# kekeliu-whu/MSF_LOAM

Measured on AMD Instinct MI355X. Metric: scan-to-map registrations/s, higher is better.
Workload: dtype f64 (f32 kNN distances)

## Files before the change

msf_loam_amd/csrc/msfl_api.hip:

```cpp
#include <hip/hip_runtime.h>
#include <rocprim/device/device_radix_sort.hpp>
#include <rocprim/device/device_scan.hpp>
#include <rocprim/device/device_select.hpp>

#include <algorithm>
#include <cmath>
#include <cstdio>
#include <cstdlib>
#include <cstring>
#include <functional>
#include <utility>
#include <chrono>
#include <string>
#include <vector>

#include <condition_variable>
#include <mutex>
#include <thread>

#include "../../include/msfl_c_api.h"
#include "msfl_kernels.cuh"
#include "msfl_extract.cuh"
#include "msfl_odom.cuh"
#include "msfl_grid.cuh"
// ... 163 lines not shown
  DevBuf rec;
  DevBuf d2, nn;
  DevBuf scan;
};

enum TimerClass { T_ASSOC = 0, T_SOLVE, T_INDEX, T_EXTRACT, T_ODOM, T_FIT, T_ASSOC_SEEDED , T_COUNT };

struct TimedSpan { hipEvent_t a, b; int cls; };

struct RejectOptions {
  int mode = MSFL_REJECT_OFF;
  double thr2 = 0.0, fraction = 0.0;
  int which = MSFL_REJECT_LAST_OUTER;
};
struct RegOptions {
  double unc_min_eig = 0.0;
  int degen_on = 0;
  double degen_min_eig = 0.0;
  RejectOptions rej;
};
struct RecordSink {
  void* out = nullptr;
  int capacity = 0;
  msfl_mem mem = MSFL_MEM_HOST;
  DevBuf dev;
  void set(const void* p, int n, msfl_mem m) { out = const_cast<void*>(p); capacity = p ? n : 0; mem = m; }
  bool host() const { return out && mem == MSFL_MEM_HOST; }
};

}

struct msfl_handle_s {
  int device = 0;
  hipStream_t own_stream = nullptr;
  hipStream_t stream = nullptr;
  msfl_params prm{};
  std::string last_error;

  bool have_map = false;
  MapIndex map_c, map_s;
  int grid_cap_cells = 64 * 1024 * 1024;
  int h2d_chunk_scans = 512;
  int h2d_sub_chunks = 2;
  int solve_records_block = 0;
  int vox_nonfinite_cloud = -1;
  const float4* vox_staged_pts = nullptr;
  bool voxel_no_big = false;
  int odom_bin_split = -1;
  int prep_split = -1;
  bool voxel_force_global = false;
  long long odom_wave_max_targets = -1;
  bool odom_force_brute = false;
  int knn_form = 0;

  DevBuf in_corner, in_surf, in_off, poses, status, info, records, pprime, nn;
  std::vector<int> in_off_host; const void* in_off_host_ptr = nullptr;
  DevBuf idx_cell_of, idx_count, idx_scanned, idx_bbox, idx_cub, idx_stage;
  bool index_single = false;
  DevBuf knn_count;
  size_t idx_count_zero = 0;
  DeskewScratch dk;
  ExtractScratch ex;
  OdomScratch od;
  VoxelScratch vox;
  PointPassScratch pp;
  PairScratch pr;
  ScoreScratch sc;

  RegOptions opt;
  RecordSink unc, degen, rej, prior;
  DevBuf rej_keys;

  PinRing pin;
  PinBuf readback;
  hipStream_t copy_stream = nullptr;
  hipEvent_t copy_ev[9] = {};

  int timing = 0;
  std::vector<TimedSpan> spans;
  std::vector<hipEvent_t> free_events;
  double t_ms[T_COUNT] = {0};
  int t_n[T_COUNT] = {0};
};

namespace {

msfl_status fail(msfl_handle* h, msfl_status s, const std::string& msg) {
  if (h) h->last_error = msg;
  return s;
}

#define HIPCHK(h, expr)                                                                            \
  do {                                                                                             \
    hipError_t e__ = (expr);                                                                       \
    if (e__ != hipSuccess)                                                                         \
      return fail(h, MSFL_HIP_ERROR, std::string(#expr) + ": " + hipGetErrorString(e__));          \
  } while (0)

msfl_status fail(msfl_places* p, msfl_status s, const std::string& msg);

template <class H, class T>
msfl_status stage_in(H* h, DevBuf& buf, const void* src, size_t n, msfl_mem mem, hipStream_t st, T** d) {
  if (mem != MSFL_MEM_HOST) { *d = static_cast<T*>(const_cast<void*>(src)); return MSFL_OK; }
  HIPCHK(h, buf.reserve(std::max<size_t>(1, n) * sizeof(T)));
  if (n > 0) HIPCHK(h, hipMemcpyAsync(buf.p, src, n * sizeof(T), hipMemcpyHostToDevice, st));
  *d = buf.as<T>();
// ... 302 lines not shown
  }
  const size_t span = (size_t)j.cap[0] + 1 + (size_t)j.cap[1] + 1;
  HIPCHK(h, h->idx_cell_of.reserve(((size_t)n_c + (size_t)n_s) * sizeof(int)));
  const void* count_before = h->idx_count.p;
  HIPCHK(h, h->idx_count.reserve(span * sizeof(int)));
  if (h->idx_count.p != count_before) h->idx_count_zero = 0;
  HIPCHK(h, h->idx_scanned.reserve(span * sizeof(int)));
  j.cell_of = h->idx_cell_of.as<int>(); j.count = h->idx_count.as<int>(); j.scanned = h->idx_scanned.as<int>();
  j.blocks0 = div_up(n_c, 256); j.bbox_blocks0 = std::min(div_up(n_c, 1024), 256);
  j.radius = std::sqrt((double)h->prm.map_knn_max_sq_dist);
  const int bbox_blocks1 = std::min(div_up(n_s, 1024), 256), blocks1 = div_up(n_s, 256);
  hipLaunchKernelGGL(grid_bbox_pair_kernel, dim3(j.bbox_blocks0 + bbox_blocks1), dim3(256), 0, st, j);
  const size_t zeroed = h->idx_count_zero;
  h->idx_count_zero = 0;
  if (span > zeroed) HIPCHK(h, hipMemsetAsync(h->idx_count.p, 0, span * sizeof(int), st));
  hipLaunchKernelGGL(grid_count_pair_kernel, dim3(j.blocks0 + blocks1), dim3(256), 0, st, j);
  size_t tmp_bytes = 0;
  HIPCHK(h, rocprim::exclusive_scan(nullptr, tmp_bytes, j.count, j.scanned, 0, span, rocprim::plus<int>(), st));
  HIPCHK(h, h->idx_cub.reserve(tmp_bytes));
  HIPCHK(h, rocprim::exclusive_scan(h->idx_cub.p, tmp_bytes, j.count, j.scanned, 0, span, rocprim::plus<int>(), st));
  hipLaunchKernelGGL(grid_scatter_pair_kernel, dim3(j.blocks0 + blocks1), dim3(256), 0, st, j);
  HIPCHK(h, hipGetLastError());
  h->idx_count_zero = std::max(zeroed, span);
  return MSFL_OK;
}

template <class Kernel, class... Tail>
void launch_knn5(msfl_handle* h, Kernel kernel, dim3 grid, dim3 block, const BatchView& bv, const double* d_poses, const int* d_status,
                 Tail... tail) {
  hipLaunchKernelGGL(kernel, grid, block, 0, h->stream, bv, d_poses, d_status,
                     (const GridDesc*)h->map_c.gdesc.as<GridDesc>(), h->map_c.sorted.as<float4>(), h->map_c.cell_start.as<int>(),
                     (const GridDesc*)h->map_s.gdesc.as<GridDesc>(), h->map_s.sorted.as<float4>(), h->map_s.cell_start.as<int>(),
                     (const int*)h->map_c.pos_of.as<int>(), (const int*)h->map_s.pos_of.as<int>(), h->prm.map_knn_max_sq_dist, tail...);
}

bool assoc_whole_batch(const msfl_handle* h, const BatchView& bv, bool deskew, int n_rec, const double* full) {
  return !deskew && !bv.dyn && n_rec >= 65536 && !full && h->timing != 3;
}

void s_launch_assoc(msfl_handle* h, const BatchView& bv_all, const double* d_poses, const int* d_status, bool deskew,
                    const DeskewView& dv, int n_rec, double* full = nullptr, int rec_begin = 0, int rec_end = -1, bool second_pass = false) {
  const bool whole_batch = rec_end < 0 && assoc_whole_batch(h, bv_all, deskew, n_rec, full);
  hipStream_t st = h->stream;
  int* nn = h->nn.as<int>();
  BatchView bv = bv_all;
  if (rec_end >= 0) { bv.rec_begin = rec_begin; bv.n_records = rec_end; n_rec = rec_end - rec_begin; }
  if (n_rec <= 0) return;
  const dim3 grid(div_up(n_rec, kAssocBlock)), block(kAssocBlock);
  {
    ScopedTimer timer(h, second_pass ? T_ASSOC_SEEDED : T_ASSOC);
    if (h->timing == 3) {
      unsigned long long* cnt = h->knn_count.as<unsigned long long>();
      if (deskew) launch_knn5(h, knn5_scan2map_kernel<true, true>, grid, block, bv, d_poses, d_status, dv, nn, cnt, nullptr, nullptr);
      else launch_knn5(h, knn5_scan2map_kernel<false, true>, grid, block, bv, d_poses, d_status, dv, nn, cnt + (second_pass ? 1 : 0), nullptr, nullptr);
    } else if (whole_batch) {
      const int n_s = bv.n_surf_total, n_c = n_rec - n_s;
      const int edge_blocks = div_up(n_c, kAssocBlock), plane_blocks = div_up(n_s, kAssocBlock);
      launch_knn5(h, knn5_scan2map_split_kernel, dim3(edge_blocks + plane_blocks), block, bv, d_poses, d_status, nn, h->records.as<double>(), edge_blocks);
    } else if (!deskew && (h->knn_form == 2 || (h->knn_form == 0 && (n_rec <= kKnnRowsMaxRecords ||
                                                                       (bv.dyn && n_rec <= 8 * kKnnRowsMaxRecords)))))
      launch_knn5(h, knn5_scan2map_rows_kernel, dim3(div_up(n_rec, kKnnRowsBlock / kKnnRowLanes)), dim3(kKnnRowsBlock), bv, d_poses, d_status, nn);
    else if (deskew)
      launch_knn5(h, knn5_scan2map_kernel<true>, grid, block, bv, d_poses, d_status, dv, nn, nullptr, nullptr, nullptr);
    else
      launch_knn5(h, knn5_scan2map_kernel<false>, grid, block, bv, d_poses, d_status, dv, nn, nullptr, nullptr, nullptr);
  }
  {
    ScopedTimer timer(h, T_FIT);
    if (deskew)
      hipLaunchKernelGGL(fit_scan2map_kernel<true>, grid, block, 0, st, bv, h->map_c.sorted.as<float4>(),
                         h->map_s.sorted.as<float4>(), (const int*)nn, h->prm.line_eigen_ratio, h->prm.plane_tolerance, dv,
                         h->records.as<double>(), full);
    else
      if (whole_batch) {
        const int n_c = n_rec - bv.n_surf_total, n_s = bv.n_surf_total;
        const int edge_blocks = div_up(n_c, kAssocBlock), plane_blocks = div_up(n_s, kAssocBlock);
        hipLaunchKernelGGL(fit_scan2map_split_kernel, dim3(edge_blocks + plane_blocks), block, 0, st, bv, h->map_c.sorted.as<float4>(),
                           h->map_s.sorted.as<float4>(), (const int*)nn, h->prm.line_eigen_ratio, h->prm.plane_tolerance, dv,
                           h->records.as<double>(), full, edge_blocks);
      } else
      hipLaunchKernelGGL(fit_scan2map_kernel<false>, grid, block, 0, st, bv, h->map_c.sorted.as<float4>(),
                         h->map_s.sorted.as<float4>(), (const int*)nn, h->prm.line_eigen_ratio, h->prm.plane_tolerance, dv,
                         h->records.as<double>(), full);
  }
}

msfl_status match_scan2map_device(msfl_handle* h, int B, const float4* d_corner, const int* h_corner_off, const float4* d_surf,
                                  const int* h_surf_off, double* d_poses, int* d_status, const RegSinks& sinks, const DeskewView* deskew,
                                  int n_chunks = 1, const int* chunk_b = nullptr, hipEvent_t* chunk_ev = nullptr,
                                  const std::function<hipError_t(int)>* enqueue_chunk = nullptr) {
  int n_rec = 0;
  { const msfl_status us = upload_batch_offsets(h, B, h_corner_off, h_surf_off, &n_rec); if (us) return us; }
  HIPCHK(h, h->records.reserve(record_bytes((size_t)n_rec, (size_t)(h_surf_off[B] - h_surf_off[0]))));
  const BatchView bv = batch_view(d_corner, d_surf, h->in_off.as<int>(), B + 1, B, n_rec, h_corner_off[0], h_surf_off[0], h_surf_off[B] - h_surf_off[0]);
  const bool nn_corner_only = n_chunks == 1 && !enqueue_chunk && assoc_whole_batch(h, bv, deskew != nullptr, n_rec, nullptr);
  HIPCHK(h, h->nn.reserve(std::max<size_t>(1, (size_t)(nn_corner_only ? n_rec - bv.n_surf_total : n_rec)) * 5 * sizeof(int)));
  DeskewView dv{};
  if (deskew) {
    dv = *deskew;
    HIPCHK(h, h->pprime.reserve(std::max<size_t>(1, (size_t)n_rec) * 3 * sizeof(double)));
    dv.pprime = h->pprime.as<double>();
  }
  const auto rec_at = [&](int b) { return h_corner_off[b] - h_corner_off[0] + h_surf_off[b] - h_surf_off[0]; };
  int longest = 0;
  for (int b = 0; b < B; b++) longest = std::max(longest, rec_at(b + 1) - rec_at(b));
  return solve_outer<kLmBlock>(h, B, bv, dv.pprime, d_poses, d_status, sinks, solver_params(h->prm, 0), h->prm.outer_iterations, [&](int it) -> msfl_status {
    if (it == 0 && (n_chunks > 1 || enqueue_chunk)) {
      for (int c = 0; c < n_chunks; c++) {
        if (enqueue_chunk) HIPCHK(h, (*enqueue_chunk)(c));
        HIPCHK(h, hipStreamWaitEvent(h->stream, chunk_ev[c], 0));
        s_launch_assoc(h, bv, d_poses, d_status, deskew != nullptr, dv, n_rec, nullptr, rec_at(chunk_b[c]), rec_at(chunk_b[c + 1]));
// ... 33 lines not shown
  p->max_sharp_per_sector = 2;
  p->max_less_sharp_per_sector = 20;
  p->max_flat_per_sector = 4;
  p->odom_distance_sq_threshold = 25.0;
  p->odom_nearby_scan = 2.5;
  p->odom_min_correspondences = 10;
  p->map_knn = 5;
  p->map_knn_max_sq_dist = 1.0f;
  p->line_eigen_ratio = 3.0;
  p->plane_tolerance = 0.2;
  p->outer_iterations = 2;
  p->max_lm_iterations = 6;
  p->huber_delta = 0.1;
  p->initial_trust_region_radius = 1e4;
  p->max_trust_region_radius = 1e16;
  p->min_trust_region_radius = 1e-32;
  p->min_relative_decrease = 1e-3;
  p->min_lm_diagonal = 1e-6;
  p->max_lm_diagonal = 1e32;
  p->function_tolerance = 1e-6;
  p->gradient_tolerance = 1e-10;
  p->parameter_tolerance = 1e-8;
  p->max_consecutive_invalid_steps = 5;
}

int msfl_api_version(void) { return MSFL_API_VERSION; }

msfl_status msfl_create(const msfl_params* params, int device, msfl_handle** out) {
  if (!out) return MSFL_BAD_ARG;
  *out = nullptr;
  int ndev = 0;
  if (hipGetDeviceCount(&ndev) != hipSuccess || ndev <= 0) return MSFL_HIP_ERROR;
  if (device < 0 || device >= ndev) return MSFL_BAD_ARG;
  msfl_handle* h = new msfl_handle_s();
  h->device = device;
  if (params) h->prm = *params; else msfl_default_params(&h->prm);
  if (h->prm.map_knn != 5 || h->prm.outer_iterations < 1 || h->prm.outer_iterations > 2 ||
      h->prm.max_lm_iterations < 0 || !(h->prm.map_knn_max_sq_dist > 0.f) ||
      h->prm.sectors_per_ring < 1 || h->prm.sectors_per_ring > 16) {
    delete h;
    return MSFL_BAD_ARG;
  }
  if (hipSetDevice(device) != hipSuccess || hipStreamCreateWithFlags(&h->own_stream, hipStreamNonBlocking) != hipSuccess) {
    delete h;
    return MSFL_HIP_ERROR;
  }
  h->stream = h->own_stream;
  if (const char* e = std::getenv("MSFL_GRID_CAP_CELLS")) { const int c = std::atoi(e); if (c >= 8 && c <= (1 << 28)) h->grid_cap_cells = c; }
  if (const char* e = std::getenv("MSFL_H2D_CHUNK_SCANS")) { const int c = std::atoi(e); if (c >= 1) h->h2d_chunk_scans = c; }
  if (const char* e = std::getenv("MSFL_H2D_SUB_CHUNKS")) { const int c = std::atoi(e); if (c >= 1) h->h2d_sub_chunks = c; }
  if (const char* e = std::getenv("MSFL_SOLVE_RECORDS_BLOCK")) h->solve_records_block = std::atoi(e);
  if (const char* e = std::getenv("MSFL_ODOM_BRUTE")) h->odom_force_brute = std::atoi(e) != 0;
  if (const char* e = std::getenv("MSFL_INDEX_SINGLE")) h->index_single = std::atoi(e) != 0;
  if (const char* e = std::getenv("MSFL_KNN_FORM")) h->knn_form = !std::strcmp(e, "lane") ? 1 : !std::strcmp(e, "rows") ? 2 : 0;
  if (const char* e = std::getenv("MSFL_ODOM_WAVE_MAX_TARGETS")) h->odom_wave_max_targets = std::atoll(e);
  if (const char* e = std::getenv("MSFL_VOXEL_GLOBAL")) h->voxel_force_global = std::atoi(e) != 0;
  if (const char* e = std::getenv("MSFL_VOXEL_NO_BIG")) h->voxel_no_big = std::atoi(e) != 0;
  if (const char* e = std::getenv("MSFL_ODOM_BIN_SPLIT")) h->odom_bin_split = std::atoi(e) != 0 ? 1 : 0;
  if (const char* e = std::getenv("MSFL_PREP_SPLIT")) { const int g = std::atoi(e); if (g == 1 || g == 2 || g == 4 || g == 8 || g == 16) h->prep_split = g; }
  *out = h;
  return MSFL_OK;
}

void msfl_destroy(msfl_handle* h) {
  if (!h) return;
#ifdef MSFL_LM_PROFILE
  {
    unsigned long long v[8] = {0};
    (void)hipDeviceSynchronize();
    (void)hipMemcpyFromSymbol(v, HIP_SYMBOL(msfl::g_lm_prof), sizeof(v));
    if (v[5]) fprintf(stderr, "[lm profile] per solve (100 MHz ticks): eval %.0f reduce %.0f serial %.0f total %.0f passes %.2f solves %llu\n",
                      (double)v[0] / v[5], (double)v[1] / v[5], (double)v[2] / v[5], (double)v[3] / v[5], (double)v[4] / v[5], v[5]);
    if (v[5]) fprintf(stderr, "[lm profile] lane-0 logic: tr_decide %.0f tr_propose %.0f ticks per solve\n", (double)v[6] / v[5], (double)v[7] / v[5]);
  }
#endif
  (void)hipSetDevice(h->device);
  (void)hipStreamSynchronize(h->stream);
  collect_timing(h);
  for (auto e : h->free_events) (void)hipEventDestroy(e);
  if (h->copy_stream) { (void)hipStreamDestroy(h->copy_stream); for (auto e : h->copy_ev) if (e) (void)hipEventDestroy(e); }
  if (h->own_stream) (void)hipStreamDestroy(h->own_stream);
  delete h;
}

msfl_status msfl_set_stream(msfl_handle* h, void* hip_stream) {
  msfl_status s = enter(h); if (s) return s;
  HIPCHK(h, hipStreamSynchronize(h->stream));
  h->stream = reinterpret_cast<hipStream_t>(hip_stream);
  return MSFL_OK;
}

msfl_status msfl_reset_stream(msfl_handle* h) {
  msfl_status s = enter(h); if (s) return s;
  HIPCHK(h, hipStreamSynchronize(h->stream));
  h->stream = h->own_stream;
  return MSFL_OK;
}

msfl_status msfl_synchronize(msfl_handle* h) {
  msfl_status s = enter(h); if (s) return s;
  HIPCHK(h, hipStreamSynchronize(h->stream));
  return MSFL_OK;
}

msfl_status msfl_set_uncertainty(msfl_handle* h, msfl_match_uncertainty* out, int capacity, msfl_mem mem, double min_eigenvalue) {
  msfl_status s = enter(h); if (s) return s;
// ... 338 lines not shown
```

msf_loam_amd/csrc/msfl_kernels.cuh:

```cuda
#pragma once
#include <hip/hip_runtime.h>
#include <stdint.h>

#include "msfl_math.cuh"
#include "msfl_record_tiles.h"
#include "msfl_knn_index.cuh"

namespace msfl {


struct FitOut { d3 C, N; bool ok; };

__device__ __forceinline__ FitOut edge_fit(const float4 (&nb)[5], double ratio) {
  FitOut o; o.ok = false; o.C = mk3(0, 0, 0); o.N = mk3(0, 0, 0);
  d3 m[5];
  d3 c = mk3(0, 0, 0);
#pragma unroll
  for (int j = 0; j < 5; j++) { m[j] = mk3((double)nb[j].x, (double)nb[j].y, (double)nb[j].z); c = c + m[j]; }
  c = mk3(c.x / 5.0, c.y / 5.0, c.z / 5.0);
  sym3 S = {0, 0, 0, 0, 0, 0};
#pragma unroll
  for (int j = 0; j < 5; j++) {
    const d3 d = m[j] - c;
    S.a00 += d.x * d.x; S.a01 += d.x * d.y; S.a02 += d.x * d.z;
// ... 61 lines not shown
__device__ __forceinline__ int find_scan_wave(const int* __restrict__ rec_off, int n_scans, int g) {
  const int g0 = __builtin_amdgcn_readfirstlane(g);
  int b = __builtin_amdgcn_readfirstlane(find_scan(rec_off, n_scans, g0));
  while (b + 1 < n_scans && g >= rec_off[b + 1]) b++;
  return b;
}
__device__ __forceinline__ int find_scan(const int* __restrict__ rec_off, int n_scans, int g) {
  int lo = 0, hi = n_scans;
  while (hi - lo > 1) {
    const int mid = (lo + hi) >> 1;
    if (rec_off[mid] <= g) lo = mid; else hi = mid;
  }
  return lo;
}

__device__ __forceinline__ size_t corner_slot(const BatchView& bv, int f) { return (size_t)(f - bv.c0); }

__device__ __forceinline__ size_t plane_slot(const BatchView& bv, int fi_surf) { return (size_t)(fi_surf - bv.s0); }
__device__ __forceinline__ size_t edge_rec_off(const BatchView& bv, int fi_corner) {
  return rec_edge((size_t)bv.n_surf_total, (size_t)(fi_corner - bv.c0));
}
__device__ __forceinline__ void plane_rec_load(const double* rec, size_t g, double (&r)[4]) {
  const double2 a = *(const double2*)(rec + rec_tile_xy(g)), b = *(const double2*)(rec + rec_tile_zc(g));
  r[0] = a.x; r[1] = a.y; r[2] = b.x; r[3] = b.y;
}
__device__ __forceinline__ void plane_rec_store(double* rec, size_t g, double nx, double ny, double nz, double d0) {
  *(double2*)(rec + rec_tile_xy(g)) = make_double2(nx, ny);
  *(double2*)(rec + rec_tile_zc(g)) = make_double2(nz, d0);
}
__device__ __forceinline__ void plane_nn_store(double* rec, size_t g, int p0, int p1, int p2, int p3, int p4) {
  char* t = (char*)rec;
  *(int4*)(t + rec_tile_nn4(g)) = make_int4(p0, p1, p2, p3);
  *(int*)(t + rec_tile_nn1(g)) = p4;
}
__device__ __forceinline__ void plane_nn_load(const double* rec, size_t g, int (&p)[5]) {
  const char* t = (const char*)rec;
  const int4 a = *(const int4*)(t + rec_tile_nn4(g));
  p[0] = a.x; p[1] = a.y; p[2] = a.z; p[3] = a.w; p[4] = *(const int*)(t + rec_tile_nn1(g));
}

struct DeskewView {
  const double* corner_dq; const double* corner_dp;
  const double* surf_dq;   const double* surf_dp;
  const double* V;
  double G[3];
  const double* G_dev;
  double* pprime;
};

#ifndef MSFL_ASSOC_BLOCK
#define MSFL_ASSOC_BLOCK 64
#endif
constexpr int kAssocBlock = MSFL_ASSOC_BLOCK;
template <bool DESKEW, bool COUNT = false, bool PAIRS = false>
__global__ void __launch_bounds__(kAssocBlock)
knn5_scan2map_kernel(BatchView bv, const double* __restrict__ poses, const int* __restrict__ status,
                     const GridDesc* __restrict__ gcp, const float4* __restrict__ map_c, const int* __restrict__ cs_c,
                     const GridDesc* __restrict__ gsp, const float4* __restrict__ map_s, const int* __restrict__ cs_s,
                     const int* __restrict__ pos_c, const int* __restrict__ pos_s,
                     float max_sq_dist, DeskewView dv, int* __restrict__ nn, unsigned long long* __restrict__ n_candidates = nullptr,
                     const int* __restrict__ cbase_c = nullptr, const int* __restrict__ cbase_s = nullptr) {
  const int g = bv.rec_begin + blockIdx.x * blockDim.x + threadIdx.x;
  if (g >= batch_records(bv)) return;
  const int b = find_scan_wave(bv.rec_off, bv.n_scans, g);
  int* out = nn + 5 * (size_t)g;
  if (status[b] != 0) { out[0] = -1; out[1] = -1; out[2] = -1; out[3] = -1; out[4] = -1; return; }
  const int local = g - bv.rec_off[b];
  const int nc = bv.corner_off[b + 1] - bv.corner_off[b];
  const bool is_edge = local < nc;
  const int fi = is_edge ? bv.corner_off[b] + local : bv.surf_off[b] + (local - nc);
  const float4 f = is_edge ? bv.corner[fi] : bv.surf[fi];
  const pose7 T = load_pose(poses + 7 * b);
  float3 q;
  if (DESKEW) {
    const double* dqp = is_edge ? dv.corner_dq + 4 * (size_t)fi : dv.surf_dq + 4 * (size_t)fi;
    const double* dpp = is_edge ? dv.corner_dp + 3 * (size_t)fi : dv.surf_dp + 3 * (size_t)fi;
    quat dq; dq.x = dqp[0]; dq.y = dqp[1]; dq.z = dqp[2]; dq.w = dqp[3];
    const d3 dp = mk3(dpp[0], dpp[1], dpp[2]);
    const double dt = (double)f.w;
    const double* Vb = dv.V + 3 * (size_t)b;
    const double Gv[3] = {dv.G_dev ? dv.G_dev[0] : dv.G[0], dv.G_dev ? dv.G_dev[1] : dv.G[1], dv.G_dev ? dv.G_dev[2] : dv.G[2]};
    const d3 shift = mk3(Vb[0] * dt - 0.5 * Gv[0] * dt * dt, Vb[1] * dt - 0.5 * Gv[1] * dt * dt,
                         Vb[2] * dt - 0.5 * Gv[2] * dt * dt);
    quat qc; qc.x = -T.q.x; qc.y = -T.q.y; qc.z = -T.q.z; qc.w = T.q.w;
    pose7 full;
    full.t = quat_rotate(T.q, quat_rotate(qc, shift) + dp) + T.t;
    full.q = quat_normalized(quat_mul(T.q, dq));
    q = transform_point_f32(full, f.x, f.y, f.z);
    const d3 pp = quat_rotate(dq, mk3((double)f.x, (double)f.y, (double)f.z)) + dp;
    dv.pprime[3 * (size_t)g + 0] = pp.x; dv.pprime[3 * (size_t)g + 1] = pp.y; dv.pprime[3 * (size_t)g + 2] = pp.z;
  } else {
    q = transform_point_f32(T, f.x, f.y, f.z);
  }
  Top5 t;
  int n_cand = 0;
  __shared__ int s_slot[kTopSlots * kAssocBlock];
  Top6K tk;
  top_init(tk, max_sq_dist, s_slot + threadIdx.x);
  if (is_edge) { const GridDesc gc = gcp[PAIRS ? b : 0]; knn5_grid_k32<kAssocBlock>(gc, map_c, cs_c, q, tk, n_cand, PAIRS ? cbase_c[b] : 0); }
  else { const GridDesc gs = gsp[PAIRS ? b : 0]; knn5_grid_k32<kAssocBlock>(gs, map_s, cs_s, q, tk, n_cand, PAIRS ? cbase_s[b] : 0); }
  const bool settled = top_settled(tk, max_sq_dist);
  if (!settled) {
    int n_again = 0;
    top5_init(t, max_sq_dist);
    if (is_edge) { const GridDesc gc = gcp[PAIRS ? b : 0]; knn5_grid(gc, map_c, cs_c + (PAIRS ? cbase_c[b] : 0), q, t, n_again); }
    else { const GridDesc gs = gsp[PAIRS ? b : 0]; knn5_grid(gs, map_s, cs_s + (PAIRS ? cbase_s[b] : 0), q, t, n_again); }
  }
  if (COUNT) {
    const unsigned long long act = __ballot(1);
    unsigned long long m = act;
    int tot = 0;
    while (m) { const int l = __ffsll((long long)m) - 1; tot += __shfl(n_cand, l); m &= m - 1; }
    if ((int)(threadIdx.x & 63) == __ffsll((long long)act) - 1) atomicAdd(n_candidates, (unsigned long long)tot);
  }
  if (settled) {
    if (top_found(tk)) {
      out[0] = top_pos<kAssocBlock>(tk, tk.k0); out[1] = top_pos<kAssocBlock>(tk, tk.k1); out[2] = top_pos<kAssocBlock>(tk, tk.k2);
      out[3] = top_pos<kAssocBlock>(tk, tk.k3); out[4] = top_pos<kAssocBlock>(tk, tk.k4);
    } else {
      out[0] = -1; out[1] = -1; out[2] = -1; out[3] = -1; out[4] = -1;
    }
    return;
  }
  if ((unsigned int)t.k4 != 0xffffffffu && (double)top5_d4(t) < (double)max_sq_dist) {
    const int* po = is_edge ? pos_c : pos_s;
    out[0] = po[(unsigned int)t.k0]; out[1] = po[(unsigned int)t.k1]; out[2] = po[(unsigned int)t.k2];
    out[3] = po[(unsigned int)t.k3]; out[4] = po[(unsigned int)t.k4];
  } else {
    out[0] = -1; out[1] = -1; out[2] = -1; out[3] = -1; out[4] = -1;
  }
}

template <class V>
__device__ __forceinline__ V uniform_load(const V* p) {
  return *(const __attribute__((address_space(4))) V*)(unsigned long long)p;
}

template <bool EDGE>
__device__ __forceinline__ void knn5_one_kind(const BatchView& bv, const double* __restrict__ poses, const int* __restrict__ status,
                                              const GridDesc* __restrict__ gp, const float4* __restrict__ map, const int* __restrict__ cs,
                                              const int* __restrict__ po, float max_sq_dist, int* __restrict__ nn, double* __restrict__ rec, int block, int* s_slot) {
  const int* off = EDGE ? bv.corner_off : bv.surf_off;
  const int f_i = off[0] + block * (int)blockDim.x + (int)threadIdx.x;
  if (f_i >= off[bv.n_scans]) return;
  const int b0 = __builtin_amdgcn_readfirstlane(find_scan(off, bv.n_scans, __builtin_amdgcn_readfirstlane(f_i)));
  int b, st; pose7 T;
  if (__all(f_i < off[b0 + 1])) {
    b = b0;
    st = uniform_load(status + b0);
    const double* pp = poses + 7 * b0;
    T.t = mk3(uniform_load(pp), uniform_load(pp + 1), uniform_load(pp + 2));
    T.q.x = uniform_load(pp + 3); T.q.y = uniform_load(pp + 4); T.q.z = uniform_load(pp + 5); T.q.w = uniform_load(pp + 6);
  } else {
    b = b0;
    while (b + 1 < bv.n_scans && f_i >= off[b + 1]) b++;
    st = status[b];
    T = load_pose(poses + 7 * b);
  }
  auto put = [&](int p0, int p1, int p2, int p3, int p4) __attribute__((always_inline)) {
    if (EDGE) { int* out = nn + 5 * corner_slot(bv, f_i); out[0] = p0; out[1] = p1; out[2] = p2; out[3] = p3; out[4] = p4; }
    else plane_nn_store(rec, plane_slot(bv, f_i), p0, p1, p2, p3, p4);
  };
  if (st != 0) { put(-1, -1, -1, -1, -1); return; }
  const float4 f = EDGE ? bv.corner[f_i] : bv.surf[f_i];
  const float3 q = transform_point_f32(T, f.x, f.y, f.z);
  int n_cand = 0;
  const GridDesc gd = *gp;
  Top6K tk;
  top_init(tk, max_sq_dist, s_slot + threadIdx.x);
  knn5_grid_k32<kAssocBlock>(gd, map, cs, q, tk, n_cand);
  if (top_settled(tk, max_sq_dist)) {
    if (top_found(tk)) {
      put(top_pos<kAssocBlock>(tk, tk.k0), top_pos<kAssocBlock>(tk, tk.k1), top_pos<kAssocBlock>(tk, tk.k2),
          top_pos<kAssocBlock>(tk, tk.k3), top_pos<kAssocBlock>(tk, tk.k4));
    } else {
      put(-1, -1, -1, -1, -1);
    }
    return;
  }
  Top5 t;
  top5_init(t, max_sq_dist);
  knn5_grid(gd, map, cs, q, t, n_cand);
  if ((unsigned int)t.k4 != 0xffffffffu && (double)top5_d4(t) < (double)max_sq_dist) {
    put(po[(unsigned int)t.k0], po[(unsigned int)t.k1], po[(unsigned int)t.k2], po[(unsigned int)t.k3], po[(unsigned int)t.k4]);
  } else {
    put(-1, -1, -1, -1, -1);
  }
}
__global__ void __launch_bounds__(kAssocBlock)
knn5_scan2map_split_kernel(BatchView bv, const double* __restrict__ poses, const int* __restrict__ status,
                           const GridDesc* __restrict__ gcp, const float4* __restrict__ map_c, const int* __restrict__ cs_c,
                           const GridDesc* __restrict__ gsp, const float4* __restrict__ map_s, const int* __restrict__ cs_s,
                           const int* __restrict__ pos_c, const int* __restrict__ pos_s, float max_sq_dist, int* __restrict__ nn,
                           double* __restrict__ rec, int edge_blocks) {
  __shared__ int s_slot[kTopSlots * kAssocBlock];
  if ((int)blockIdx.x < edge_blocks) knn5_one_kind<true>(bv, poses, status, gcp, map_c, cs_c, pos_c, max_sq_dist, nn, rec, (int)blockIdx.x, s_slot);
  else knn5_one_kind<false>(bv, poses, status, gsp, map_s, cs_s, pos_s, max_sq_dist, nn, rec, (int)blockIdx.x - edge_blocks, s_slot);
}

constexpr int kKnnRowLanes = 16;
constexpr int kKnnRowsBlock = 256;
#ifndef MSFL_KNN_ROWS_MAX
#define MSFL_KNN_ROWS_MAX 32768
#endif
constexpr int kKnnRowsMaxRecords = MSFL_KNN_ROWS_MAX;
__global__ void __launch_bounds__(kKnnRowsBlock)
knn5_scan2map_rows_kernel(BatchView bv, const double* __restrict__ poses, const int* __restrict__ status,
                          const GridDesc* __restrict__ gcp, const float4* __restrict__ map_c, const int* __restrict__ cs_c,
                          const GridDesc* __restrict__ gsp, const float4* __restrict__ map_s, const int* __restrict__ cs_s,
                          const int* __restrict__ pos_c, const int* __restrict__ pos_s, float max_sq_dist, int* __restrict__ nn) {
  const int sl = threadIdx.x & (kKnnRowLanes - 1);
  const int g = bv.rec_begin + (int)((blockIdx.x * kKnnRowsBlock + threadIdx.x) / kKnnRowLanes);
  if (g >= batch_records(bv)) return;
  const int b = find_scan(bv.rec_off, bv.n_scans, g);
  int* out = nn + 5 * (size_t)g;
  if (status[b] != 0) { if (sl < 5) out[sl] = -1; return; }
  const int local = g - bv.rec_off[b];
  const int nc = bv.corner_off[b + 1] - bv.corner_off[b];
  const bool is_edge = local < nc;
  const int fi = is_edge ? bv.corner_off[b] + local : bv.surf_off[b] + (local - nc);
  const float4 f = is_edge ? bv.corner[fi] : bv.surf[fi];
  const pose7 T = load_pose(poses + 7 * b);
  const float3 q = transform_point_f32(T, f.x, f.y, f.z);
  const GridDesc gd = is_edge ? *gcp : *gsp;
  const float4* __restrict__ sorted = is_edge ? map_c : map_s;
  const int* __restrict__ cell_start = is_edge ? cs_c : cs_s;
  Top5 t;
  top5_init(t, max_sq_dist);
  const unsigned long long sentinel = t.k0;
  const GridQuery w = grid_query(gd, q);
  const int y = w.cy + (sl % 3) - 1, z = w.cz + (sl / 3) - 1;
  if (sl < 9 && w.xs <= w.xe && y >= 0 && y < gd.dy && z >= 0 && z < gd.dz) {
    const float gy = axis_gap(w.uy, y), gz = axis_gap(w.uz, z);
    const float row2 = (gy * gy + gz * gz) * gd.cell2;
    if (!(row2 > max_sq_dist)) {
      float gxa[kGridXSub], gxb[kGridXSub];
      grid_x_bounds(gd, w, gxa, gxb);
      int a = w.xs, e_cell = w.xe;
      bool da = true, db = true;
#pragma unroll
      for (int k = 0; k < kGridXSub; k++) {
        da = da && (row2 + gxa[k] > max_sq_dist); a += da ? 1 : 0;
        db = db && (row2 + gxb[k] > max_sq_dist); e_cell -= db ? 1 : 0;
      }
      if (a <= e_cell) {
        const int row = (z * gd.dy + y) * gd.dx;
        const int s = cell_start[row + a], e = cell_start[row + e_cell + 1];
        const msfl_f2 qxy = {q.x, q.y};
        for (int i = s; i < e; i += 4) {
          float4 m[4];
// ... 628 lines not shown
```

msf_loam_amd/csrc/msfl_knn_index.cuh:

```cuda
#pragma once
#include <hip/hip_runtime.h>
#include <stdint.h>

#include "msfl_math.cuh"

namespace msfl {

#ifndef MSFL_GRID_XSUB
#define MSFL_GRID_XSUB 3
#endif
constexpr int kGridXSub = MSFL_GRID_XSUB;

struct GridDesc {
  float ox, oy, oz;
  float inv_cell;
  float inv_cell_x;
  int dx, dy, dz;
  int n_pts;
  int n_cells;
  int reach;
  int want_cells;
  float cell2, cellx2;
};

// ... 364 lines not shown
      const bool e = (r == 6) == o.e_first;
      dy = e ? sy : -sy; dz = e ? -sz : sz; gy = e ? o.g_ny : o.g_fy; gz = e ? o.g_fz : o.g_nz;
    } else { dy = -sy; dz = -sz; gy = o.g_fy; gz = o.g_fz; }
    const int y = w.cy + dy, z = w.cz + dz;
    if (y < 0 || y >= g.dy || z < 0 || z >= g.dz) continue;
    const float row2 = (gy * gy + gz * gz) * g.cell2;
    const int row = (z * g.dy + y) * g.dx;
    const float d = bound();
    if (row2 > d) continue;
    int a = w.xs, b = w.xe;
    bool da = true, db = true;
#pragma unroll
    for (int k = 0; k < kGridXSub; k++) {
      da = da && (row2 + gxa[k] > d); a += da ? 1 : 0;
      db = db && (row2 + gxb[k] > d); b -= db ? 1 : 0;
    }
    if (a > b) continue;
    scan(cell_start[row + a], cell_start[row + b + 1]);
  }
}

__device__ __forceinline__ void knn5_grid(const GridDesc& g, const float4* __restrict__ sorted,
                                          const int* __restrict__ cell_start, float3 q, Top5& t,
                                          int& n_cand) {
  const msfl_f2 qxy = {q.x, q.y};
  grid_walk_exact(g, cell_start, q, [&]() __attribute__((always_inline)) { return top5_d4(t); },
                  [&](int s, int e) __attribute__((always_inline)) {
    n_cand += e - s;
    const float4* p = sorted + s;
    const float4* const pe = sorted + e;
    for (; p + 1 < pe; p += 2) {
      float4 m0 = p[0], m1 = p[1];
      asm volatile("" : "+v"(m0.w));
      top5_insert(t, l2_simple_pk(m0, qxy, q.z), __float_as_int(m0.w));
      asm volatile("" : "+v"(m1.w));
      top5_insert(t, l2_simple_pk(m1, qxy, q.z), __float_as_int(m1.w));
    }
    if (p < pe) { float4 m = p[0]; asm volatile("" : "+v"(m.w)); top5_insert(t, l2_simple_pk(m, qxy, q.z), __float_as_int(m.w)); }
  });
}

template <int STRIDE>
__device__ __forceinline__ void top_insert_off(Top6K& t, float d, unsigned int off) {
  const unsigned int db = __float_as_uint(d);
  if (db > t.bound) return;
  const unsigned int slot = t.k5 & 7u;
  const unsigned int x = (db & ~7u) | slot;
  t.col[slot * STRIDE] = (int)off;
  u32_med3_into(t.k5, t.k4, x); u32_med3_into(t.k4, t.k3, x); u32_med3_into(t.k3, t.k2, x);
  u32_med3_into(t.k2, t.k1, x); u32_med3_into(t.k1, t.k0, x);
  t.k0 = min(t.k0, x);
  t.bound = min(t.k4 | 7u, t.gate);
}
template <int STRIDE>
__device__ __forceinline__ void knn5_grid_k32(const GridDesc& g, const float4* __restrict__ sorted,
                                              const int* __restrict__ cell_start, float3 q, Top6K& t, int& n_cand,
                                              int cell_base = 0) {
  const GridQuery w = grid_query(g, q);
  const int cy = w.cy, cz = w.cz, xs = w.xs, xe = w.xe;
  if (xs > xe) return;
  const float cell2 = g.cell2;
  float gxa[kGridXSub], gxb[kGridXSub];
  grid_x_bounds<true>(g, w, gxa, gxb);
  const msfl_f2 qxy = {q.x, q.y};
  const GridRowOrder o = grid_row_order(w);
  const float q_ny = o.g_ny * o.g_ny, q_fy = o.g_fy * o.g_fy, q_nz = o.g_nz * o.g_nz, q_fz = o.g_fz * o.g_fz, q_y1 = o.gy1 * o.gy1, q_z1 = o.gz1 * o.gz1;
  const int sy = o.sy, sz = o.sz;
  const bool v_y1 = (unsigned int)cy < (unsigned int)g.dy, v_ny = (unsigned int)(cy + sy) < (unsigned int)g.dy, v_fy = (unsigned int)(cy - sy) < (unsigned int)g.dy;
  const bool v_z1 = (unsigned int)cz < (unsigned int)g.dz, v_nz = (unsigned int)(cz + sz) < (unsigned int)g.dz, v_fz = (unsigned int)(cz - sz) < (unsigned int)g.dz;
  const int base0 = (cz * g.dy + cy) * g.dx + cell_base;
  const int off_y = sy < 0 ? -g.dx : g.dx;
  const int zstep = g.dy * g.dx;
  const int off_z = sz < 0 ? -zstep : zstep;
  const char* const mapb = (const char*)sorted;
  auto visit = [&](bool valid, int row, float rowq) __attribute__((always_inline)) {
    const float row2 = rowq * cell2;
    const float d4 = top_d4(t);
    if (!valid || row2 > d4) return;
    const float room = d4 - row2;
    int a = xs, b = xe;
#pragma unroll
    for (int k = 0; k < kGridXSub; k++) { a += gxa[k] > room ? 1 : 0; b -= gxb[k] > room ? 1 : 0; }
    if (a > b) return;
    const unsigned int s = (unsigned int)cell_start[(unsigned int)(row + a)], e = (unsigned int)cell_start[(unsigned int)(row + b + 1)];
    if (s == e) return;
    n_cand += (int)(e - s);
    unsigned int off = s << 4;
    const unsigned int end = e << 4, last = end - 16u;
    for (; off < last; off += 32u) {
      float4 m0 = *(const float4*)(mapb + off), m1 = *(const float4*)(mapb + off + 16u);
      asm volatile("" : "+v"(m0.w));
      top_insert_off<STRIDE>(t, l2_simple_pk(m0, qxy, q.z), off);
      asm volatile("" : "+v"(m1.w));
      top_insert_off<STRIDE>(t, l2_simple_pk(m1, qxy, q.z), off + 16u);
    }
    if (off < end) { float4 m = *(const float4*)(mapb + off); asm volatile("" : "+v"(m.w)); top_insert_off<STRIDE>(t, l2_simple_pk(m, qxy, q.z), off); }
  };
  visit(v_y1 && v_z1, base0, q_y1 + q_z1);
  {
    const bool va = v_ny && v_z1, vb = v_y1 && v_nz;
    const float ra = q_ny + q_z1, rb = q_y1 + q_nz;
    visit(o.ny_first ? va : vb, base0 + (o.ny_first ? off_y : off_z), o.ny_first ? ra : rb);
    visit(o.ny_first ? vb : va, base0 + (o.ny_first ? off_z : off_y), o.ny_first ? rb : ra);
  }
  {
    const bool va = v_fy && v_z1, vb = v_y1 && v_fz;
    const float ra = q_fy + q_z1, rb = q_y1 + q_fz;
    visit(o.fy_first ? va : vb, base0 - (o.fy_first ? off_y : off_z), o.fy_first ? ra : rb);
    visit(o.fy_first ? vb : va, base0 - (o.fy_first ? off_z : off_y), o.fy_first ? rb : ra);
  }
  visit(v_ny && v_nz, base0 + off_y + off_z, q_ny + q_nz);
  {
    const bool va = v_ny && v_fz, vb = v_fy && v_nz;
    const float ra = q_ny + q_fz, rb = q_fy + q_nz;
    const int oa = off_y - off_z, ob = off_z - off_y;
    visit(o.e_first ? va : vb, base0 + (o.e_first ? oa : ob), o.e_first ? ra : rb);
    visit(o.e_first ? vb : va, base0 + (o.e_first ? ob : oa), o.e_first ? rb : ra);
  }
  visit(v_fy && v_fz, base0 - off_y - off_z, q_fy + q_fz);
}

}
```

Measured before the change: 1.024 million.

## Defer long kNN grid row tails to a second flat pass

Each visited grid row segment is cut at a per-position cap, and the remainder is pushed onto a small per-thread stack in shared memory. After all nine rows are visited with a tighter top-5 bound, the deferred tails are scanned in one flat loop. The aim is to shrink the kNN bound early so later row pruning skips more candidates, and to reduce lane divergence from uneven row lengths. In exchange it uses more shared memory per block and adds stack bookkeeping. The deferred tails are still scanned in full, so results are unchanged.

```diff
diff --git a/msf_loam_amd/csrc/msfl_api.hip b/msf_loam_amd/csrc/msfl_api.hip
--- a/msf_loam_amd/csrc/msfl_api.hip
+++ b/msf_loam_amd/csrc/msfl_api.hip
@@ -239,6 +239,7 @@
   long long odom_wave_max_targets = -1;
   bool odom_force_brute = false;
   int knn_form = 0;
+  bool knn_defer = true;
 
   DevBuf in_corner, in_surf, in_off, poses, status, info, records, pprime, nn;
   std::vector<int> in_off_host; const void* in_off_host_ptr = nullptr;
@@ -647,11 +648,14 @@
     if (h->timing == 3) {
       unsigned long long* cnt = h->knn_count.as<unsigned long long>();
       if (deskew) launch_knn5(h, knn5_scan2map_kernel<true, true>, grid, block, bv, d_poses, d_status, dv, nn, cnt, nullptr, nullptr);
+      else if (h->knn_defer) launch_knn5(h, knn5_scan2map_kernel<false, true, false, true>, grid, block, bv, d_poses, d_status, dv, nn, cnt + (second_pass ? 1 : 0), nullptr, nullptr);
       else launch_knn5(h, knn5_scan2map_kernel<false, true>, grid, block, bv, d_poses, d_status, dv, nn, cnt + (second_pass ? 1 : 0), nullptr, nullptr);
     } else if (whole_batch) {
       const int n_s = bv.n_surf_total, n_c = n_rec - n_s;
       const int edge_blocks = div_up(n_c, kAssocBlock), plane_blocks = div_up(n_s, kAssocBlock);
-      launch_knn5(h, knn5_scan2map_split_kernel, dim3(edge_blocks + plane_blocks), block, bv, d_poses, d_status, nn, h->records.as<double>(), edge_blocks);
+      const dim3 blocks(edge_blocks + plane_blocks);
+      if (h->knn_defer) launch_knn5(h, knn5_scan2map_split_kernel<true>, blocks, block, bv, d_poses, d_status, nn, h->records.as<double>(), edge_blocks);
+      else launch_knn5(h, knn5_scan2map_split_kernel<false>, blocks, block, bv, d_poses, d_status, nn, h->records.as<double>(), edge_blocks);
     } else if (!deskew && (h->knn_form == 2 || (h->knn_form == 0 && (n_rec <= kKnnRowsMaxRecords ||
                                                                        (bv.dyn && n_rec <= 8 * kKnnRowsMaxRecords)))))
       launch_knn5(h, knn5_scan2map_rows_kernel, dim3(div_up(n_rec, kKnnRowsBlock / kKnnRowLanes)), dim3(kKnnRowsBlock), bv, d_poses, d_status, nn);
@@ -791,6 +795,7 @@
   if (const char* e = std::getenv("MSFL_SOLVE_RECORDS_BLOCK")) h->solve_records_block = std::atoi(e);
   if (const char* e = std::getenv("MSFL_ODOM_BRUTE")) h->odom_force_brute = std::atoi(e) != 0;
   if (const char* e = std::getenv("MSFL_INDEX_SINGLE")) h->index_single = std::atoi(e) != 0;
+  if (const char* e = std::getenv("MSFL_KNN_DEFER")) h->knn_defer = std::atoi(e) != 0;
   if (const char* e = std::getenv("MSFL_KNN_FORM")) h->knn_form = !std::strcmp(e, "lane") ? 1 : !std::strcmp(e, "rows") ? 2 : 0;
   if (const char* e = std::getenv("MSFL_ODOM_WAVE_MAX_TARGETS")) h->odom_wave_max_targets = std::atoll(e);
   if (const char* e = std::getenv("MSFL_VOXEL_GLOBAL")) h->voxel_force_global = std::atoi(e) != 0;
diff --git a/msf_loam_amd/csrc/msfl_kernels.cuh b/msf_loam_amd/csrc/msfl_kernels.cuh
--- a/msf_loam_amd/csrc/msfl_kernels.cuh
+++ b/msf_loam_amd/csrc/msfl_kernels.cuh
@@ -137,7 +137,7 @@
 #define MSFL_ASSOC_BLOCK 64
 #endif
 constexpr int kAssocBlock = MSFL_ASSOC_BLOCK;
-template <bool DESKEW, bool COUNT = false, bool PAIRS = false>
+template <bool DESKEW, bool COUNT = false, bool PAIRS = false, bool DEFER = false>
 __global__ void __launch_bounds__(kAssocBlock)
 knn5_scan2map_kernel(BatchView bv, const double* __restrict__ poses, const int* __restrict__ status,
                      const GridDesc* __restrict__ gcp, const float4* __restrict__ map_c, const int* __restrict__ cs_c,
@@ -179,11 +179,11 @@
   }
   Top5 t;
   int n_cand = 0;
-  __shared__ int s_slot[kTopSlots * kAssocBlock];
+  __shared__ int s_slot[(kTopSlots + (DEFER ? kDeferSlots : 0)) * kAssocBlock];
   Top6K tk;
   top_init(tk, max_sq_dist, s_slot + threadIdx.x);
-  if (is_edge) { const GridDesc gc = gcp[PAIRS ? b : 0]; knn5_grid_k32<kAssocBlock>(gc, map_c, cs_c, q, tk, n_cand, PAIRS ? cbase_c[b] : 0); }
-  else { const GridDesc gs = gsp[PAIRS ? b : 0]; knn5_grid_k32<kAssocBlock>(gs, map_s, cs_s, q, tk, n_cand, PAIRS ? cbase_s[b] : 0); }
+  if (is_edge) { const GridDesc gc = gcp[PAIRS ? b : 0]; knn5_grid_k32<kAssocBlock, DEFER>(gc, map_c, cs_c, q, tk, n_cand, PAIRS ? cbase_c[b] : 0); }
+  else { const GridDesc gs = gsp[PAIRS ? b : 0]; knn5_grid_k32<kAssocBlock, DEFER>(gs, map_s, cs_s, q, tk, n_cand, PAIRS ? cbase_s[b] : 0); }
   const bool settled = top_settled(tk, max_sq_dist);
   if (!settled) {
     int n_again = 0;
@@ -221,7 +221,7 @@
   return *(const __attribute__((address_space(4))) V*)(unsigned long long)p;
 }
 
-template <bool EDGE>
+template <bool EDGE, bool DEFER>
 __device__ __forceinline__ void knn5_one_kind(const BatchView& bv, const double* __restrict__ poses, const int* __restrict__ status,
                                               const GridDesc* __restrict__ gp, const float4* __restrict__ map, const int* __restrict__ cs,
                                               const int* __restrict__ po, float max_sq_dist, int* __restrict__ nn, double* __restrict__ rec, int block, int* s_slot) {
@@ -253,7 +253,7 @@
   const GridDesc gd = *gp;
   Top6K tk;
   top_init(tk, max_sq_dist, s_slot + threadIdx.x);
-  knn5_grid_k32<kAssocBlock>(gd, map, cs, q, tk, n_cand);
+  knn5_grid_k32<kAssocBlock, DEFER>(gd, map, cs, q, tk, n_cand);
   if (top_settled(tk, max_sq_dist)) {
     if (top_found(tk)) {
       put(top_pos<kAssocBlock>(tk, tk.k0), top_pos<kAssocBlock>(tk, tk.k1), top_pos<kAssocBlock>(tk, tk.k2),
@@ -272,15 +272,16 @@
     put(-1, -1, -1, -1, -1);
   }
 }
+template <bool DEFER>
 __global__ void __launch_bounds__(kAssocBlock)
 knn5_scan2map_split_kernel(BatchView bv, const double* __restrict__ poses, const int* __restrict__ status,
                            const GridDesc* __restrict__ gcp, const float4* __restrict__ map_c, const int* __restrict__ cs_c,
                            const GridDesc* __restrict__ gsp, const float4* __restrict__ map_s, const int* __restrict__ cs_s,
                            const int* __restrict__ pos_c, const int* __restrict__ pos_s, float max_sq_dist, int* __restrict__ nn,
                            double* __restrict__ rec, int edge_blocks) {
-  __shared__ int s_slot[kTopSlots * kAssocBlock];
-  if ((int)blockIdx.x < edge_blocks) knn5_one_kind<true>(bv, poses, status, gcp, map_c, cs_c, pos_c, max_sq_dist, nn, rec, (int)blockIdx.x, s_slot);
-  else knn5_one_kind<false>(bv, poses, status, gsp, map_s, cs_s, pos_s, max_sq_dist, nn, rec, (int)blockIdx.x - edge_blocks, s_slot);
+  __shared__ int s_slot[(kTopSlots + (DEFER ? kDeferSlots : 0)) * kAssocBlock];
+  if ((int)blockIdx.x < edge_blocks) knn5_one_kind<true, DEFER>(bv, poses, status, gcp, map_c, cs_c, pos_c, max_sq_dist, nn, rec, (int)blockIdx.x, s_slot);
+  else knn5_one_kind<false, DEFER>(bv, poses, status, gsp, map_s, cs_s, pos_s, max_sq_dist, nn, rec, (int)blockIdx.x - edge_blocks, s_slot);
 }
 
 constexpr int kKnnRowLanes = 16;
diff --git a/msf_loam_amd/csrc/msfl_knn_index.cuh b/msf_loam_amd/csrc/msfl_knn_index.cuh
--- a/msf_loam_amd/csrc/msfl_knn_index.cuh
+++ b/msf_loam_amd/csrc/msfl_knn_index.cuh
@@ -440,7 +440,19 @@
   t.k0 = min(t.k0, x);
   t.bound = min(t.k4 | 7u, t.gate);
 }
-template <int STRIDE>
+#ifndef MSFL_KNN_DEFER_CAPS
+#define MSFL_KNN_DEFER_CAPS 8, 4, 4, 1, 1, 1, 1, 1, 1
+#endif
+#ifndef MSFL_KNN_DEFER_DEPTH
+#define MSFL_KNN_DEFER_DEPTH 4
+#endif
+#ifndef MSFL_KNN_DEFER_FLAT
+#define MSFL_KNN_DEFER_FLAT 1
+#endif
+constexpr int kDeferCaps[9] = {MSFL_KNN_DEFER_CAPS};
+constexpr int kDeferDepth = MSFL_KNN_DEFER_DEPTH;
+constexpr int kDeferSlots = 2 * kDeferDepth;
+template <int STRIDE, bool DEFER = false>
 __device__ __forceinline__ void knn5_grid_k32(const GridDesc& g, const float4* __restrict__ sorted,
                                               const int* __restrict__ cell_start, float3 q, Top6K& t, int& n_cand,
                                               int cell_base = 0) {
@@ -461,7 +473,9 @@
   const int zstep = g.dy * g.dx;
   const int off_z = sz < 0 ? -zstep : zstep;
   const char* const mapb = (const char*)sorted;
-  auto visit = [&](bool valid, int row, float rowq) __attribute__((always_inline)) {
+  int* const stack = t.col + kTopSlots * STRIDE;
+  int* sp = stack;
+  auto visit = [&](int pos, bool valid, int row, float rowq) __attribute__((always_inline)) {
     const float row2 = rowq * cell2;
     const float d4 = top_d4(t);
     if (!valid || row2 > d4) return;
@@ -472,9 +486,19 @@
     if (a > b) return;
     const unsigned int s = (unsigned int)cell_start[(unsigned int)(row + a)], e = (unsigned int)cell_start[(unsigned int)(row + b + 1)];
     if (s == e) return;
-    n_cand += (int)(e - s);
     unsigned int off = s << 4;
-    const unsigned int end = e << 4, last = end - 16u;
+    unsigned int end = e << 4;
+    if constexpr (DEFER) {
+      const unsigned int cut = off + 32u * (unsigned int)kDeferCaps[pos];
+      if (end > cut && sp < stack + kDeferSlots * STRIDE) {
+        sp[0] = (int)cut; sp[STRIDE] = (int)end; sp += 2 * STRIDE;
+        end = cut;
+      }
+      n_cand += (int)((end - off) >> 4);
+    } else {
+      n_cand += (int)(e - s);
+    }
+    const unsigned int last = end - 16u;
     for (; off < last; off += 32u) {
       float4 m0 = *(const float4*)(mapb + off), m1 = *(const float4*)(mapb + off + 16u);
       asm volatile("" : "+v"(m0.w));
@@ -484,28 +508,61 @@
     }
     if (off < end) { float4 m = *(const float4*)(mapb + off); asm volatile("" : "+v"(m.w)); top_insert_off<STRIDE>(t, l2_simple_pk(m, qxy, q.z), off); }
   };
-  visit(v_y1 && v_z1, base0, q_y1 + q_z1);
+  visit(0, v_y1 && v_z1, base0, q_y1 + q_z1);
   {
     const bool va = v_ny && v_z1, vb = v_y1 && v_nz;
     const float ra = q_ny + q_z1, rb = q_y1 + q_nz;
-    visit(o.ny_first ? va : vb, base0 + (o.ny_first ? off_y : off_z), o.ny_first ? ra : rb);
-    visit(o.ny_first ? vb : va, base0 + (o.ny_first ? off_z : off_y), o.ny_first ? rb : ra);
+    visit(1, o.ny_first ? va : vb, base0 + (o.ny_first ? off_y : off_z), o.ny_first ? ra : rb);
+    visit(2, o.ny_first ? vb : va, base0 + (o.ny_first ? off_z : off_y), o.ny_first ? rb : ra);
   }
   {
     const bool va = v_fy && v_z1, vb = v_y1 && v_fz;
     const float ra = q_fy + q_z1, rb = q_y1 + q_fz;
-    visit(o.fy_first ? va : vb, base0 - (o.fy_first ? off_y : off_z), o.fy_first ? ra : rb);
-    visit(o.fy_first ? vb : va, base0 - (o.fy_first ? off_z : off_y), o.fy_first ? rb : ra);
-  }
-  visit(v_ny && v_nz, base0 + off_y + off_z, q_ny + q_nz);
+    visit(3, o.fy_first ? va : vb, base0 - (o.fy_first ? off_y : off_z), o.fy_first ? ra : rb);
+    visit(4, o.fy_first ? vb : va, base0 - (o.fy_first ? off_z : off_y), o.fy_first ? rb : ra);
+  }
+  visit(5, v_ny && v_nz, base0 + off_y + off_z, q_ny + q_nz);
   {
     const bool va = v_ny && v_fz, vb = v_fy && v_nz;
     const float ra = q_ny + q_fz, rb = q_fy + q_nz;
     const int oa = off_y - off_z, ob = off_z - off_y;
-    visit(o.e_first ? va : vb, base0 + (o.e_first ? oa : ob), o.e_first ? ra : rb);
-    visit(o.e_first ? vb : va, base0 + (o.e_first ? ob : oa), o.e_first ? rb : ra);
-  }
-  visit(v_fy && v_fz, base0 - off_y - off_z, q_fy + q_fz);
-}
-
-}
+    visit(6, o.e_first ? va : vb, base0 + (o.e_first ? oa : ob), o.e_first ? ra : rb);
+    visit(7, o.e_first ? vb : va, base0 + (o.e_first ? ob : oa), o.e_first ? rb : ra);
+  }
+  visit(8, v_fy && v_fz, base0 - off_y - off_z, q_fy + q_fz);
+  if constexpr (DEFER) {
+    if (MSFL_KNN_DEFER_FLAT) {
+      unsigned int off = 0, end = 0;
+      for (const int* rp = stack;; off += 32u) {
+        if (off >= end) {
+          if (rp >= sp) break;
+          off = (unsigned int)rp[0]; end = (unsigned int)rp[STRIDE]; rp += 2 * STRIDE;
+          n_cand += (int)((end - off) >> 4);
+        }
+        const bool two = off + 16u < end;
+        const unsigned int off1 = two ? off + 16u : off;
+        float4 m0 = *(const float4*)(mapb + off), m1 = *(const float4*)(mapb + off1);
+        asm volatile("" : "+v"(m0.w));
+        top_insert_off<STRIDE>(t, l2_simple_pk(m0, qxy, q.z), off);
+        asm volatile("" : "+v"(m1.w));
+        top_insert_off<STRIDE>(t, two ? l2_simple_pk(m1, qxy, q.z) : __uint_as_float(0xffffffffu), off1);
+      }
+    } else {
+      for (const int* rp = stack; rp < sp; rp += 2 * STRIDE) {
+        unsigned int off = (unsigned int)rp[0];
+        const unsigned int end = (unsigned int)rp[STRIDE], last = end - 16u;
+        n_cand += (int)((end - off) >> 4);
+        for (; off < last; off += 32u) {
+          float4 m0 = *(const float4*)(mapb + off), m1 = *(const float4*)(mapb + off + 16u);
+          asm volatile("" : "+v"(m0.w));
+          top_insert_off<STRIDE>(t, l2_simple_pk(m0, qxy, q.z), off);
+          asm volatile("" : "+v"(m1.w));
+          top_insert_off<STRIDE>(t, l2_simple_pk(m1, qxy, q.z), off + 16u);
+        }
+        if (off < end) { float4 m = *(const float4*)(mapb + off); asm volatile("" : "+v"(m.w)); top_insert_off<STRIDE>(t, l2_simple_pk(m, qxy, q.z), off); }
+      }
+    }
+  }
+}
+
+}
```

New measurement: 1.072 million (median of 6 runs). 1.05x the previous value.
